# MyNiuuu/MOFA-Video

Hardware: AMD Instinct MI355X
Metric: denoised frames/sec, 25f 576x1024 SVD+MOFA, 25 steps (higher is better)
Workload: dtype f16; 1 GPU; MOFA-Video-Traj, 25-frame 576x1024, 25 denoise steps + temporal VAE decode (chunk 8), single trajectory hint, SVD-XT UNet + MOFA-Adapter, CFG 1->3, seeded random weights in the reference checkpoint layout; num_frames=25, height=576, width=1024, num_inference_steps=25, decode_chunk_size=8, parallelism=1 GPU, graph_steps=False, output_finite=True

## Files before the change

### mofa_video_amd/csrc/attention.hip

```cpp

#include "common.h"

#define ATT_TILE 64
#define ATT_DEFER_SUM 16384.0f

typedef short att_s16x4 __attribute__((ext_vector_type(4)));
__device__ __forceinline__ f16x4 lds_read_tr4(const f16* p) {
    const att_s16x4 v = __builtin_amdgcn_ds_read_tr16_b64_v4i16((__attribute__((address_space(3))) att_s16x4*)p);
    return __builtin_bit_cast(f16x4, v);
}

template <int D, int QB>
__global__ __launch_bounds__(256, 2) void attn_spatial_kernel(const f16* __restrict__ q, const f16* __restrict__ k,
                                                              const f16* __restrict__ v, f16* __restrict__ out,
                                                              int heads, int S, int ldq, int ldk, int ldv, int ldo, float c,
                                                              int nqb, int total) {
    constexpr bool DMA = D == 64;
    constexpr int NBUF = 2;
    constexpr int ATT_KSTR = DMA ? D : D + 8;
    constexpr int ATT_VSTR = DMA ? D : D + 32;
    constexpr int KK = D / 16;
    constexpr int DB = D / 32;
    constexpr int NCH = D / 32;
    extern __shared__ __attribute__((aligned(16))) char smem_att[];
    f16* sKb = (f16*)smem_att;
    f16* sVb = sKb + NBUF * ATT_TILE * ATT_KSTR;

    const int tid = threadIdx.x, lane = tid & 63, wave = tid >> 6;
    const int l31 = lane & 31, lh = lane >> 5;
    int head, frame, qb_;
    {
        const int xcd = blockIdx.x & 7, local = blockIdx.x >> 3, qn = total >> 3, rn = total & 7;
        const int start = xcd < rn ? xcd * (qn + 1) : rn * (qn + 1) + (xcd - rn) * qn;
        if (local >= qn + (xcd < rn ? 1 : 0)) return;
        const int w = start + local, pair = w / nqb;
        qb_ = w - pair * nqb;
        frame = pair / heads;
        head = pair - frame * heads;
    }
    const int q0 = qb_ * (128 * QB) + wave * (32 * QB);

    const f16* kbase = k + (size_t)frame * S * ldk + head * D;
    const f16* vbase = v + (size_t)frame * S * ldv + head * D;

    f16x8 qf[QB][KK];
    const f16x8 zero8 = {0, 0, 0, 0, 0, 0, 0, 0};
#pragma unroll
    for (int b = 0; b < QB; ++b) {
        const int qi = q0 + b * 32 + l31;
        const f16* qp = q + ((size_t)frame * S + (qi < S ? qi : 0)) * ldq + head * D + lh * 8;
#pragma unroll
        for (int kk = 0; kk < KK; ++kk) {
            const f16x8 v = (qi < S) ? *(const f16x8*)(qp + kk * 16) : zero8;
            qf[b][kk] = v;
            if (c != 1.0f) {
#pragma unroll
                for (int e = 0; e < 8; ++e) qf[b][kk][e] = (f16)((float)v[e] * c);
            }
        }
    }

    constexpr bool NEGM = D == 64;
    f32x16 o[QB][DB];
    f32x16 negm[QB];
    float m_run[QB], l_run[QB];
#pragma unroll
    for (int b = 0; b < QB; ++b) {
#pragma unroll
        for (int r = 0; r < 16; ++r) negm[b][r] = 0.f;
        m_run[b] = 0.f; l_run[b] = 0.f;
#pragma unroll
        for (int db = 0; db < DB; ++db)
#pragma unroll
            for (int r = 0; r < 16; ++r) o[b][db][r] = 0.f;
    }

    constexpr int CPR = D / 8;
    f16x8 gk[NCH], gv[NCH];
    const f16* kptr[NCH];
    const f16* vptr[NCH];
#pragma unroll
    for (int i = 0; i < NCH; ++i) {
        const int cidx = tid + 256 * i;
        const int krow = cidx / CPR, kcol = cidx - krow * CPR;
        kptr[i] = kbase + (size_t)krow * ldk + kcol * 8;
        vptr[i] = vbase + (size_t)krow * ldv + kcol * 8;
    }
    const size_t kstep = (size_t)ATT_TILE * ldk, vstep = (size_t)ATT_TILE * ldv;
    auto load_tile = [&](int k0) {
        if (__builtin_amdgcn_readfirstlane(k0 + ATT_TILE <= S)) {
#pragma unroll
            for (int i = 0; i < NCH; ++i) {
                gk[i] = *(const f16x8*)kptr[i];
                gv[i] = *(const f16x8*)vptr[i];
            }
        } else {
#pragma unroll
            for (int i = 0; i < NCH; ++i) {
                const bool ok = k0 + (tid + 256 * i) / CPR < S;
                gk[i] = ok ? *(const f16x8*)kptr[i] : zero8;
                gv[i] = ok ? *(const f16x8*)vptr[i] : zero8;
            }
        }
#pragma unroll
        for (int i = 0; i < NCH; ++i) { kptr[i] += kstep; vptr[i] += vstep; }
    };
    auto store_tile = [&](int buf) {
        f16* sK = sKb + buf * ATT_TILE * ATT_KSTR;
        f16* sV = sVb + buf * ATT_TILE * ATT_VSTR;
#pragma unroll
        for (int i = 0; i < NCH; ++i) {
            const int cidx = tid + 256 * i;
            const int krow = cidx / CPR, kcol = cidx - krow * CPR;
            *(f16x8*)&sK[krow * ATT_KSTR + kcol * 8] = gk[i];
            *(f16x8*)&sV[krow * ATT_VSTR + kcol * 8] = gv[i];
        }
    };
    const int tr_off = (((lane & 15) >> 2) + 4 * lh) * ATT_VSTR + 16 * ((lane >> 4) & 1) + 4 * (lane & 3);

    const auto rsk = __builtin_amdgcn_make_buffer_rsrc((void*)kbase, 0, (unsigned)(((size_t)(S - 1) * ldk + D) * 2), 0x00020000);
    const auto rsv = __builtin_amdgcn_make_buffer_rsrc((void*)vbase, 0, (unsigned)(((size_t)(S - 1) * ldv + D) * 2), 0x00020000);
    unsigned dko[2], dvo[2];
#pragma unroll
    for (int i = 0; i < 2; ++i) {
        const int row = (2 * wave + i) * 8 + (lane >> 3), slot = lane & 7;
        dko[i] = (unsigned)row * (unsigned)ldk * 2u + (unsigned)((slot ^ ((row >> 1) & 7)) * 16);
        dvo[i] = (unsigned)row * (unsigned)ldv * 2u + (unsigned)((slot ^ (4 * ((row >> 1) & 1))) * 16);
    }
    auto dma_tile = [&](int t, int buf) __attribute__((always_inline)) {
        char* bk = (char*)(sKb + buf * ATT_TILE * ATT_KSTR) + (2 * wave) * 1024;
        char* bv = (char*)(sVb + buf * ATT_TILE * ATT_VSTR) + (2 * wave) * 1024;
#pragma unroll
        for (int i = 0; i < 2; ++i) {
            __builtin_amdgcn_raw_ptr_buffer_load_lds(rsk, (__attribute__((address_space(3))) void*)(bk + i * 1024), 16, dko[i],
                                                     t * ATT_TILE * ldk * 2, 0, 0);
            __builtin_amdgcn_raw_ptr_buffer_load_lds(rsv, (__attribute__((address_space(3))) void*)(bv + i * 1024), 16, dvo[i],
                                                     t * ATT_TILE * ldv * 2, 0, 0);
        }
    };
    const int ksw = (l31 >> 1) & 7;
    const int vsw = (lane >> 3) & 1;

    const int ntiles = (S + ATT_TILE - 1) / ATT_TILE;
    if constexpr (DMA) {
        dma_tile(0, 0);
        asm volatile("s_waitcnt vmcnt(0)" ::: "memory");
    } else {
        load_tile(0);
        store_tile(0);
    }
    __syncthreads();

    int buf = 0;
    for (int t = 0; t < ntiles; ++t, buf = (buf + 1 == NBUF ? 0 : buf + 1)) {
        const int k0 = t * ATT_TILE;
        if (t + 1 < ntiles) {
            if constexpr (DMA) dma_tile(t + 1, buf ^ 1);
            else load_tile(k0 + ATT_TILE);
        }

        f32x16 s[QB][2];
#pragma unroll
        for (int ts = 0; ts < 2; ++ts) {
            if constexpr (!NEGM) {
#pragma unroll
                for (int b = 0; b < QB; ++b)
#pragma unroll
                    for (int r = 0; r < 16; ++r) s[b][ts][r] = -m_run[b];
            }
            const f16* kp = sKb + buf * ATT_TILE * ATT_KSTR + (ts * 32 + l31) * ATT_KSTR + (DMA ? 0 : lh * 8);
#pragma unroll
            for (int kk = 0; kk < KK; ++kk) {
                const f16x8 kf = *(const f16x8*)(kp + (DMA ? ((2 * kk + lh) ^ ksw) * 8 : kk * 16));
#pragma unroll
                for (int b = 0; b < QB; ++b)
                    s[b][ts] = __builtin_amdgcn_mfma_f32_32x32x16_f16(kf, qf[b][kk], (NEGM && kk == 0) ? negm[b] : s[b][ts], 0, 0, 0);
            }
        }
        if (__builtin_amdgcn_readfirstlane(k0 + ATT_TILE > S)) {
            asm volatile("; tail tile" ::: "memory");
#pragma unroll
            for (int b = 0; b < QB; ++b)
#pragma unroll
                for (int ts = 0; ts < 2; ++ts)
#pragma unroll
                    for (int r = 0; r < 16; ++r) {
                        const int key = k0 + ts * 32 + (r & 3) + 8 * (r >> 2) + 4 * lh;
                        if (key >= S) s[b][ts][r] = -1e30f;
                    }
        }
        f16x8 pf[QB][2][2];
#pragma unroll
        for (int b = 0; b < QB; ++b) {
            float psum = 0.f;
#pragma unroll
            for (int ts = 0; ts < 2; ++ts)
#pragma unroll
                for (int r = 0; r < 16; ++r) {
                    const float p = __builtin_amdgcn_exp2f(s[b][ts][r]);
                    psum += p;
                    pf[b][ts][r >> 3][r & 7] = (f16)p;
                }
            const float ptot = psum + __shfl_xor(psum, 32, 64);
            const bool move = !(ptot < ATT_DEFER_SUM) || t == 0;
            if (__any(move)) {
                asm volatile("; reference moves" ::: "memory");
                float mx = s[b][0][0];
#pragma unroll
                for (int ts = 0; ts < 2; ++ts)
#pragma unroll
                    for (int r = 0; r < 16; ++r) mx = fmaxf(mx, s[b][ts][r]);
                mx = fmaxf(mx, __shfl_xor(mx, 32, 64));
                const float delta = move ? mx : 0.f;
                const float alpha = __builtin_amdgcn_exp2f(-delta);
                m_run[b] += delta;
                if constexpr (NEGM) {
#pragma unroll
                    for (int r = 0; r < 16; ++r) negm[b][r] = -m_run[b];
                }
                l_run[b] *= alpha;
#pragma unroll
                for (int db = 0; db < DB; ++db)
#pragma unroll
                    for (int r = 0; r < 16; ++r) o[b][db][r] *= alpha;
                psum = 0.f;
#pragma unroll
                for (int ts = 0; ts < 2; ++ts)
#pragma unroll
                    for (int r = 0; r < 16; ++r) {
                        const float p = __builtin_amdgcn_exp2f(s[b][ts][r] - delta);
                        psum += p;
                        pf[b][ts][r >> 3][r & 7] = (f16)p;
                    }
            }
            l_run[b] += psum;
        }

#pragma unroll
        for (int db = 0; db < DB; ++db) {
            const f16* vp = sVb + buf * ATT_TILE * ATT_VSTR + tr_off + (DMA ? (db ^ vsw) : db) * 32;
#pragma unroll
            for (int ts = 0; ts < 2; ++ts)
#pragma unroll
                for (int u = 0; u < 2; ++u) {
                    const f16x4 lo = lds_read_tr4(vp + (ts * 32 + u * 16) * ATT_VSTR);
                    const f16x4 hi = lds_read_tr4(vp + (ts * 32 + u * 16 + 8) * ATT_VSTR);
                    const f16x8 vf = {lo[0], lo[1], lo[2], lo[3], hi[0], hi[1], hi[2], hi[3]};
#pragma unroll
                    for (int b = 0; b < QB; ++b) o[b][db] = __builtin_amdgcn_mfma_f32_32x32x16_f16(vf, pf[b][ts][u], o[b][db], 0, 0, 0);
                }
        }
        if (t + 1 < ntiles) {
            if constexpr (DMA) asm volatile("s_waitcnt vmcnt(0)" ::: "memory");
            else store_tile(buf ^ 1);
        }
        __syncthreads();
    }

#pragma unroll
    for (int b = 0; b < QB; ++b) {
        const float l_tot = l_run[b] + __shfl_xor(l_run[b], 32, 64);
        const float inv = 1.0f / l_tot;
        const int qi = q0 + b * 32 + l31;
        if (qi < S) {
            f16* op = out + ((size_t)frame * S + qi) * ldo + head * D;
#pragma unroll
            for (int db = 0; db < DB; ++db)
#pragma unroll
                for (int qd = 0; qd < 4; ++qd) {
                    f16x4 v;
#pragma unroll
                    for (int e = 0; e < 4; ++e) v[e] = (f16)(o[b][db][4 * qd + e] * inv);
                    *(f16x4*)(op + db * 32 + 8 * qd + 4 * lh) = v;
                }
        }
    }
}

template <int D, int QB>
static int launch_attn_spatial(const void* q, const void* k, const void* v, void* out, int nframes, int heads, int S,
                               int ldq, int ldk, int ldv, int ldo, float c, hipStream_t st) {
    constexpr int LDS = D == 64 ? 2 * (ATT_TILE * D + ATT_TILE * D) * 2 : 2 * (ATT_TILE * (D + 8) + ATT_TILE * (D + 32)) * 2;
    const int nqb = cdiv(S, 128 * QB);
    const long long total = (long long)nqb * heads * nframes;
    if (total > 0x7ffffff0LL) return MOFA_EINVAL;
    static LaunchSetup setup;
    if (setup.cus([](int) { return mofa_lds_optin((const void*)attn_spatial_kernel<D, QB>, LDS); }) == 0) return MOFA_ELAUNCH;
    dim3 grid((unsigned)(8 * ((total + 7) / 8)));
    hipLaunchKernelGGL((attn_spatial_kernel<D, QB>), grid, dim3(256), LDS, st, (const f16*)q, (const f16*)k, (const f16*)v,
                       (f16*)out, heads, S, ldq, ldk, ldv, ldo, c, nqb, (int)total);
    MOFA_CHECK_LAUNCH();
    return MOFA_OK;
}

extern "C" int mofa_attn_spatial_qb_f16(const void* q, const void* k, const void* v, void* out, int nframes, int heads,
                                        int head_dim, int S, int ldq, int ldk, int ldv, int ldo, float scale,
                                        int query_blocks, mofa_stream_t stream) {
    if (!q || !k || !v || !out || nframes <= 0 || heads <= 0 || S <= 0) return MOFA_EINVAL;
    if (ldq % 8 != 0 || ldk % 8 != 0 || ldv % 8 != 0 || ldo % 4 != 0) return MOFA_EINVAL;
    if (query_blocks < 0 || query_blocks > 2 || (query_blocks == 2 && head_dim != 64)) return MOFA_EINVAL;
    const float c = scale > 0.f ? scale * 1.4426950408889634f : 1.0f;
    const bool two = query_blocks ? query_blocks == 2
                                  : ((long long)cdiv(S, 256) * 256 * 16 <= (long long)S * 17 && (long long)cdiv(S, 256) * heads * nframes >= 1024);
    if (head_dim == 64)
        return two ? launch_attn_spatial<64, 2>(q, k, v, out, nframes, heads, S, ldq, ldk, ldv, ldo, c, (hipStream_t)stream)
                   : launch_attn_spatial<64, 1>(q, k, v, out, nframes, heads, S, ldq, ldk, ldv, ldo, c, (hipStream_t)stream);
    if (head_dim == 128)
        return launch_attn_spatial<128, 1>(q, k, v, out, nframes, heads, S, ldq, ldk, ldv, ldo, c, (hipStream_t)stream);
    return MOFA_EINVAL;
}

extern "C" int mofa_attn_spatial_f16(const void* q, const void* k, const void* v, void* out, int nframes, int heads,
                                     int head_dim, int S, int ldq, int ldk, int ldv, int ldo, float scale,
                                     mofa_stream_t stream) {
    return mofa_attn_spatial_qb_f16(q, k, v, out, nframes, heads, head_dim, S, ldq, ldk, ldv, ldo, scale, 0, stream);
}

__global__ __launch_bounds__(256) void transpose_v_kernel(const f16* __restrict__ v, f16* __restrict__ vt, int heads,
                                                          int S, int ldv) {
    __shared__ f16 s[64][66];
    const int tid = threadIdx.x;
    const int k0 = blockIdx.x * 64, head = blockIdx.y, frame = blockIdx.z;
    {
        const int key = tid >> 2, dc = (tid & 3) * 16;
        if (k0 + key < S) {
            const f16* p = v + ((size_t)frame * S + k0 + key) * ldv + head * 64 + dc;
            const f16x8 a = *(const f16x8*)p, b = *(const f16x8*)(p + 8);
#pragma unroll
            for (int e = 0; e < 8; ++e) { s[dc + e][key] = a[e]; s[dc + 8 + e][key] = b[e]; }
        }
    }
    __syncthreads();
    {
        const int d = tid >> 2, kc = (tid & 3) * 16;
        f16* p = vt + ((size_t)(frame * heads + head) * 64 + d) * S + k0 + kc;
#pragma unroll
        for (int half = 0; half < 2; ++half) {
            if (k0 + kc + half * 8 < S) {
                f16x8 a;
#pragma unroll
                for (int e = 0; e < 8; ++e) a[e] = s[d][kc + half * 8 + e];
                *(f16x8*)(p + half * 8) = a;
            }
        }
    }
}

extern "C" int mofa_transpose_v_f16(const void* v, void* vt, int nframes, int heads, int S, int ldv,
                                    mofa_stream_t stream) {
    if (!v || !vt || nframes <= 0 || heads <= 0 || S <= 0 || S % 8 != 0 || ldv % 8 != 0) return MOFA_EINVAL;
    dim3 grid(cdiv(S, 64), heads, nframes);
    hipLaunchKernelGGL(transpose_v_kernel, grid, dim3(256), 0, (hipStream_t)stream, (const f16*)v, (f16*)vt, heads, S,
                       ldv);
    MOFA_CHECK_LAUNCH();
    return MOFA_OK;
}

template <int D, int WPB>
__global__ __launch_bounds__(64 * WPB) void attn_temporal_kernel(const f16* __restrict__ q, const f16* __restrict__ k,
                                                                 const f16* __restrict__ v, f16* __restrict__ out,
                                                                 long long nseq, int Tq, int T, int HW, int heads, int ld,
                                                                 int ldkv, int ldo, float scale, unsigned key_mask) {
    constexpr int DC = D / 8;
    constexpr int KK = D / 16;
    constexpr int DB = D / 32;
    constexpr int KSTR = D + 8;
    constexpr int VSTR = D + 32;
    __shared__ __attribute__((aligned(16))) f16 sK[WPB][32 * KSTR];
    __shared__ __attribute__((aligned(16))) f16 sV[WPB][32 * VSTR];
    const int tid = threadIdx.x, lane = tid & 63, wave = tid >> 6;
    const long long seq = (long long)blockIdx.x * WPB + wave;
    if (seq >= nseq) return;
    const int l31 = lane & 31, lh = lane >> 5;
    const int head = (int)(seq % heads);
    const long long bp = seq / heads;
    const int p = (int)(bp % HW);
    const int b = (int)(bp / HW);
    const size_t base = ((size_t)b * T * HW + p);
    const size_t qbase = ((size_t)b * Tq * HW + p);
    f16* wK = sK[wave];
    f16* wV = sV[wave];
    const f16x8 zero8 = {0, 0, 0, 0, 0, 0, 0, 0};

    for (int c = lane; c < 32 * DC; c += 64) {
        *(f16x8*)&wK[(c / DC) * KSTR + (c % DC) * 8] = zero8;
        *(f16x8*)&wV[(c / DC) * VSTR + (c % DC) * 8] = zero8;
    }
    f16x8 qf[KK];
    {
        const f16* qp = q + (qbase + (size_t)(l31 < Tq ? l31 : 0) * HW) * ld + head * D + lh * 8;
#pragma unroll
        for (int kk = 0; kk < KK; ++kk) qf[kk] = l31 < Tq ? *(const f16x8*)(qp + kk * 16) : zero8;
    }
    for (int c = lane; c < T * DC; c += 64) {
        const int t = c / DC, cc = c - t * DC;
        if (!((key_mask >> t) & 1u)) continue;
        const size_t row = base + (size_t)t * HW;
        const f16x8 kv = *(const f16x8*)(k + row * ldkv + head * D + cc * 8);
        const f16x8 vv = *(const f16x8*)(v + row * ldkv + head * D + cc * 8);
        *(f16x8*)&wK[t * KSTR + cc * 8] = kv;
        *(f16x8*)&wV[t * VSTR + cc * 8] = vv;
    }
    asm volatile("s_waitcnt lgkmcnt(0)" ::: "memory");
    __builtin_amdgcn_wave_barrier();

    f32x16 s;
#pragma unroll
    for (int r = 0; r < 16; ++r) s[r] = 0.f;
    {
        const f16* kp = wK + l31 * KSTR + lh * 8;
#pragma unroll
        for (int kk = 0; kk < KK; ++kk) {
            const f16x8 kf = *(const f16x8*)(kp + kk * 16);
            s = __builtin_amdgcn_mfma_f32_32x32x16_f16(kf, qf[kk], s, 0, 0, 0);
        }
    }
    const float c2 = scale * 1.4426950408889634f;
    float mx = -1e30f;
#pragma unroll
    for (int r = 0; r < 16; ++r) {
        const int key = (r & 3) + 8 * (r >> 2) + 4 * lh;
        if (key >= T || !((key_mask >> key) & 1u)) s[r] = -1e30f;
        mx = fmaxf(mx, s[r]);
    }
    mx = fmaxf(mx, __shfl_xor(mx, 32, 64));
    const float mc = mx * c2;
    float sum = 0.f;
    f16x8 pf[2];
#pragma unroll
    for (int r = 0; r < 16; ++r) {
        const float pr = __builtin_amdgcn_exp2f(fmaf(s[r], c2, -mc));
        sum += pr;
        pf[r >> 3][r & 7] = (f16)pr;
    }
    sum += __shfl_xor(sum, 32, 64);
    const float inv = 1.0f / sum;

    f32x16 o[DB];
#pragma unroll
    for (int db = 0; db < DB; ++db) {
#pragma unroll
        for (int r = 0; r < 16; ++r) o[db][r] = 0.f;
        const f16* vp = wV + (((lane & 15) >> 2) + 4 * lh) * VSTR + db * 32 + 16 * ((lane >> 4) & 1) + 4 * (lane & 3);
#pragma unroll
        for (int u = 0; u < 2; ++u) {
            const f16x4 lo = lds_read_tr4(vp + (u * 16) * VSTR), hi = lds_read_tr4(vp + (u * 16 + 8) * VSTR);
            const f16x8 vf = {lo[0], lo[1], lo[2], lo[3], hi[0], hi[1], hi[2], hi[3]};
            o[db] = __builtin_amdgcn_mfma_f32_32x32x16_f16(vf, pf[u], o[db], 0, 0, 0);
        }
    }
    if (l31 < Tq) {
        f16* op = out + (qbase + (size_t)l31 * HW) * ldo + head * D;
#pragma unroll
        for (int db = 0; db < DB; ++db)
#pragma unroll
            for (int qd = 0; qd < 4; ++qd) {
                f16x4 w;
#pragma unroll
                for (int e = 0; e < 4; ++e) w[e] = (f16)(o[db][4 * qd + e] * inv);
                *(f16x4*)(op + db * 32 + 8 * qd + 4 * lh) = w;
            }
    }
}

extern "C" int mofa_attn_temporal_masked_f16(const void* q, const void* k, const void* v, void* out, int nclips, int Tq,
                                             int T, int HW, int heads, int head_dim, int ld, int ldkv, int ldo, float scale,
                                             uint32_t key_mask, mofa_stream_t stream) {
    if (!q || !k || !v || !out || nclips <= 0 || T <= 0 || T > 32 || Tq <= 0 || Tq > T || HW <= 0 || heads <= 0)
        return MOFA_EINVAL;
    if (T < 32) key_mask &= (1u << T) - 1u;
    if (key_mask == 0) return MOFA_EINVAL;
    if (ld % 8 != 0 || ldkv % 8 != 0 || ldo % 8 != 0) return MOFA_EINVAL;
    const long long nseq = (long long)nclips * HW * heads;
    if (head_dim == 64) {
        hipLaunchKernelGGL((attn_temporal_kernel<64, 4>), dim3(cdiv(nseq, 4)), dim3(256), 0, (hipStream_t)stream,
                           (const f16*)q, (const f16*)k, (const f16*)v, (f16*)out, nseq, Tq, T, HW, heads, ld, ldkv, ldo, scale,
                           key_mask);
    } else if (head_dim == 128) {
        hipLaunchKernelGGL((attn_temporal_kernel<128, 2>), dim3(cdiv(nseq, 2)), dim3(128), 0, (hipStream_t)stream,
                           (const f16*)q, (const f16*)k, (const f16*)v, (f16*)out, nseq, Tq, T, HW, heads, ld, ldkv, ldo, scale,
                           key_mask);
    } else {
        return MOFA_EINVAL;
    }
    MOFA_CHECK_LAUNCH();
    return MOFA_OK;
}

extern "C" int mofa_attn_temporal_f16(const void* q, const void* k, const void* v, void* out, int nclips, int Tq, int T,
                                      int HW, int heads, int head_dim, int ld, int ldkv, int ldo, float scale,
                                      mofa_stream_t stream) {
    return mofa_attn_temporal_masked_f16(q, k, v, out, nclips, Tq, T, HW, heads, head_dim, ld, ldkv, ldo, scale, 0xffffffffu,
                                         stream);
}

#define TL_SLOT(r) (((r) & 3) + 8 * ((r) >> 2))

template <int D, int KT, int WPB>
__global__ __launch_bounds__(64 * WPB) void attn_temporal_long_kernel(const f16* __restrict__ q, const f16* __restrict__ k,
                                                                      const f16* __restrict__ v, f16* __restrict__ out,
                                                                      long long nseq, int T, int HW, int heads, int ld,
                                                                      int ldkv, int ldo, float scale) {
#define TL_TQ T
#define TL_STAGE_WORD(t0)
#define TL_STAGED(t) ((t) < T)
#define TL_WORDS(q0)
#define TL_HIDDEN(kt, r) ((kt) == KT - 1 && (kt) * 32 + TL_SLOT(r) + 4 * lh >= T)
#include "attn_temporal_long_body.inc"
}

template <int D, int KT, int WPB>
__global__ __launch_bounds__(64 * WPB) void attn_temporal_long_masked_kernel(const f16* __restrict__ q, const f16* __restrict__ k,
                                                                             const f16* __restrict__ v, f16* __restrict__ out,
                                                                             long long nseq, int Tq, int T, int HW, int heads,
                                                                             int ld, int ldkv, int ldo, float scale, unsigned m0,
                                                                             unsigned m1, unsigned m2, unsigned m3) {
#define TL_MASK_WORD(w) ((w) == 0 ? m0 : (w) == 1 ? m1 : (w) == 2 ? m2 : m3)
#define TL_TQ Tq
#define TL_STAGE_WORD(t0) const unsigned mw = TL_MASK_WORD((t0) >> 5);
#define TL_STAGED(t) ((mw >> ((t) & 31)) & 1u)
#define TL_WORDS(q0)                    \
    unsigned ml[KT];                    \
    _Pragma("unroll") for (int kt = 0; kt < KT; ++kt) ml[kt] = (TL_MASK_WORD(kt) >> (4 * lh)) | (unsigned)((q0) >> 20);
#define TL_HIDDEN(kt, r) (!(ml[kt] & (1u << TL_SLOT(r))))
#include "attn_temporal_long_body.inc"
#undef TL_MASK_WORD
}

template <int D, int KT, int WPB>
__global__ __launch_bounds__(64 * WPB) void attn_temporal_long_local_kernel(const f16* __restrict__ q, const f16* __restrict__ k,
                                                                            const f16* __restrict__ v, f16* __restrict__ out,
                                                                            long long nseq, int T, int HW, int heads, int ld,
                                                                            int ldkv, int ldo, float scale, int radius,
                                                                            int anchor) {
#define TL_TQ T
#define TL_STAGE_WORD(t0)
#define TL_STAGED(t) ((t) < T)
#define TL_WORDS(q0)                                                                                                \
    const int qi = min((q0) + l31, T - 1);                                                                          \
    const int lo = max(qi - radius, 0), hi1 = min(qi + radius, T - 1) + 1;                                          \
    unsigned ml[KT];                                                                                                \
    _Pragma("unroll") for (int kt = 0; kt < KT; ++kt) {                                                             \
        const auto below = [](int n) { return (unsigned)((1ull << min(max(n, 0), 32)) - 1ull); };                   \
        ml[kt] = (below(anchor - 32 * kt) | (below(hi1 - 32 * kt) & ~below(lo - 32 * kt))) >> (4 * lh);             \
    }
#define TL_HIDDEN(kt, r) (!(ml[kt] & (1u << TL_SLOT(r))))
#include "attn_temporal_long_body.inc"
}

template <int D, int KT, int WPB>
__global__ __launch_bounds__(64 * WPB) void attn_temporal_long_window_kernel(const f16* __restrict__ q, const f16* __restrict__ k,
                                                                             const f16* __restrict__ v, f16* __restrict__ out,
                                                                             long long nseq, int Tq, int T, int HW, int heads,
                                                                             int ld, int ldkv, int ldo, float scale, int radius,
                                                                             int anchor, int q_frame0, int band_frame0) {
#define TL_TQ Tq
#define TL_STAGE_WORD(t0)
#define TL_STAGED(t) ((t) < T)
#define TL_WORDS(q0)                                                                                                \
    const int g = q_frame0 + min((q0) + l31, Tq - 1);                                                               \
    const int lo = anchor + max(max(g - radius, anchor), band_frame0) - band_frame0;                                \
    const int hi1 = anchor + min(g + radius, band_frame0 + (T - anchor) - 1) - band_frame0 + 1;                     \
    unsigned ml[KT];                                                                                                \
    _Pragma("unroll") for (int kt = 0; kt < KT; ++kt) {                                                             \
        const auto below = [](int n) { return (unsigned)((1ull << min(max(n, 0), 32)) - 1ull); };                   \
        ml[kt] = (below(anchor - 32 * kt) | (below(hi1 - 32 * kt) & ~below(lo - 32 * kt))) >> (4 * lh);             \
    }
#define TL_HIDDEN(kt, r) (!(ml[kt] & (1u << TL_SLOT(r))))
#include "attn_temporal_long_body.inc"
}

template <int D>
struct TemporalStreamTile {
    static constexpr int DC = D / 8, KSTR = D + 8, VSTR = D + 32, RPI = 64 / DC, N = 32 / RPI;
    f16x8 gk[N], gv[N];
    __device__ __forceinline__ void load(const f16* __restrict__ k, const f16* __restrict__ v, size_t base, int HW, int ldkv, int head,
                                         int T, int t_first, int lane) {
        const f16x8 zero8 = {0, 0, 0, 0, 0, 0, 0, 0};
        const int r0 = lane / DC, cc = lane % DC;
#pragma unroll
        for (int u = 0; u < N; ++u) {
            const int t = t_first + u * RPI + r0;
            gk[u] = zero8; gv[u] = zero8;
            if (t < T) {
                const size_t off = (base + (size_t)t * HW) * ldkv + head * D + cc * 8;
                gk[u] = *(const f16x8*)(k + off);
                gv[u] = *(const f16x8*)(v + off);
            }
        }
    }
    __device__ __forceinline__ void store(f16* rk, f16* rv, int lane) const {
        const int r0 = lane / DC, cc = lane % DC;
#pragma unroll
        for (int u = 0; u < N; ++u) {
            const int i = u * RPI + r0;
            *(f16x8*)&rk[i * KSTR + cc * 8] = gk[u];
            *(f16x8*)&rv[i * VSTR + cc * 8] = gv[u];
        }
    }
};

template <int D, int WPB>
__global__ __launch_bounds__(64 * WPB) void attn_temporal_stream_local_kernel(const f16* __restrict__ q, const f16* __restrict__ k,
                                                                              const f16* __restrict__ v, f16* __restrict__ out,
                                                                              long long nseq, int T, int HW, int heads, int ld,
                                                                              int ldkv, int ldo, float scale, int radius,
                                                                              int anchor) {
    constexpr int KK = D / 16, DB = D / 32, KSTR = D + 8, VSTR = D + 32;
    constexpr int NS = 4, ROWS = 32 * NS;
    extern __shared__ __attribute__((aligned(16))) char smem_ts[];
    const int tid = threadIdx.x, lane = tid & 63, wave = tid >> 6;
    const long long seq = (long long)blockIdx.x * WPB + wave;
    if (seq >= nseq) return;
    const int l31 = lane & 31, lh = lane >> 5;
    const int head = (int)(seq % heads);
    const long long bp = seq / heads;
    const int p = (int)(bp % HW);
    const int b = (int)(bp / HW);
    const size_t base = ((size_t)b * T * HW + p);
    f16* wK = (f16*)smem_ts + (size_t)wave * (ROWS * (KSTR + VSTR));
    f16* wV = wK + ROWS * KSTR;
    const f16x8 zero8 = {0, 0, 0, 0, 0, 0, 0, 0};

    f16x8 qf[KK];
    {
        const f16* qp = q + (base + (size_t)(l31 < T ? l31 : 0) * HW) * ld + head * D + lh * 8;
#pragma unroll
        for (int kk = 0; kk < KK; ++kk) qf[kk] = l31 < T ? *(const f16x8*)(qp + kk * 16) : zero8;
    }
    {
        TemporalStreamTile<D> t0, t1, tz;
        t0.load(k, v, base, HW, ldkv, head, T, 0, lane);
        t1.load(k, v, base, HW, ldkv, head, T, 32, lane);
        tz.load(k, v, base, HW, ldkv, head, T, T, lane);
        t0.store(wK, wV, lane);
        t1.store(wK + 64 * KSTR, wV + 64 * VSTR, lane);
        tz.store(wK + 32 * KSTR, wV + 32 * VSTR, lane);
        tz.store(wK + 96 * KSTR, wV + 96 * VSTR, lane);
    }
    asm volatile("s_waitcnt lgkmcnt(0)" ::: "memory");
    __builtin_amdgcn_wave_barrier();

    const float c2 = scale * 1.4426950408889634f;
    const int tr_off = (((lane & 15) >> 2) + 4 * lh) * VSTR + 16 * ((lane >> 4) & 1) + 4 * (lane & 3);
    int sa = 3, sb = 1, sc = 2;
#pragma unroll 1
    for (int q0 = 0; q0 < T; q0 += 32) {
        const int tq = q0 >> 5;
        const int slot[NS] = {0, sa, sb, sc};
        TemporalStreamTile<D> nt;
        nt.load(k, v, base, HW, ldkv, head, T, q0 + 64, lane);
        f16x8 qn[KK];
        {
            const int qi = q0 + 32 + l31;
            const f16* qp = q + (base + (size_t)(qi < T ? qi : 0) * HW) * ld + head * D + lh * 8;
#pragma unroll
            for (int kk = 0; kk < KK; ++kk) qn[kk] = qi < T ? *(const f16x8*)(qp + kk * 16) : zero8;
        }
        unsigned ml[NS];
        {
            const int qi = min(q0 + l31, T - 1);
            const int lo = max(qi - radius, 0), hi1 = min(qi + radius, T - 1) + 1;
            const auto below = [](int n) { return (unsigned)((1ull << min(max(n, 0), 32)) - 1ull); };
            ml[0] = (below(anchor) | (below(hi1) & ~below(lo))) >> (4 * lh);
#pragma unroll
            for (int j = 1; j < NS; ++j) {
                const int tt = tq + j - 2;
                const unsigned band = below(hi1 - 32 * tt) & ~below(lo - 32 * tt);
                ml[j] = (tt == 0 ? 0u : band) >> (4 * lh);
            }
        }
        f32x16 s[NS];
#pragma unroll
        for (int j = 0; j < NS; ++j) {
#pragma unroll
            for (int r = 0; r < 16; ++r) s[j][r] = 0.f;
            const f16* kp = wK + (slot[j] * 32 + l31) * KSTR + lh * 8;
#pragma unroll
            for (int kk = 0; kk < KK; ++kk) {
                const f16x8 kf = *(const f16x8*)(kp + kk * 16);
                s[j] = __builtin_amdgcn_mfma_f32_32x32x16_f16(kf, qf[kk], s[j], 0, 0, 0);
            }
        }
        float mx = -1e30f;
#pragma unroll
        for (int j = 0; j < NS; ++j)
#pragma unroll
            for (int r = 0; r < 16; ++r) {
                if (!(ml[j] & (1u << TL_SLOT(r)))) s[j][r] = -1e30f;
                mx = fmaxf(mx, s[j][r]);
            }
        mx = fmaxf(mx, __shfl_xor(mx, 32, 64));
        const float mc = mx * c2;
        float sum = 0.f;
        f16x8 pf[NS][2];
#pragma unroll
        for (int j = 0; j < NS; ++j)
#pragma unroll
            for (int r = 0; r < 16; ++r) {
                const float pr = __builtin_amdgcn_exp2f(fmaf(s[j][r], c2, -mc));
                sum += pr;
                pf[j][r >> 3][r & 7] = (f16)pr;
            }
        sum += __shfl_xor(sum, 32, 64);
        const float inv = 1.0f / sum;

        f32x16 o[DB];
#pragma unroll
        for (int db = 0; db < DB; ++db) {
#pragma unroll
            for (int r = 0; r < 16; ++r) o[db][r] = 0.f;
            const f16* vp = wV + tr_off + db * 32;
#pragma unroll
            for (int j = 0; j < NS; ++j)
#pragma unroll
                for (int u = 0; u < 2; ++u) {
                    const f16x4 lo = lds_read_tr4(vp + (slot[j] * 32 + u * 16) * VSTR), hi = lds_read_tr4(vp + (slot[j] * 32 + u * 16 + 8) * VSTR);
                    const f16x8 vf = {lo[0], lo[1], lo[2], lo[3], hi[0], hi[1], hi[2], hi[3]};
                    o[db] = __builtin_amdgcn_mfma_f32_32x32x16_f16(vf, pf[j][u], o[db], 0, 0, 0);
                }
        }
        asm volatile("s_waitcnt lgkmcnt(0)" ::: "memory");
        __builtin_amdgcn_wave_barrier();
        nt.store(wK + sa * 32 * KSTR, wV + sa * 32 * VSTR, lane);
        asm volatile("s_waitcnt lgkmcnt(0)" ::: "memory");
        __builtin_amdgcn_wave_barrier();
        if (q0 + l31 < T) {
            f16* op = out + (base + (size_t)(q0 + l31) * HW) * ldo + head * D;
#pragma unroll
            for (int db = 0; db < DB; ++db)
#pragma unroll
                for (int qd = 0; qd < 4; ++qd) {
                    f16x4 w;
#pragma unroll
                    for (int e = 0; e < 4; ++e) w[e] = (f16)(o[db][4 * qd + e] * inv);
                    *(f16x4*)(op + db * 32 + 8 * qd + 4 * lh) = w;
                }
        }
        const int s0 = sa;
        sa = sb; sb = sc; sc = s0;
#pragma unroll
        for (int kk = 0; kk < KK; ++kk) qf[kk] = qn[kk];
    }
}
#undef TL_SLOT

template <int D_, int KT_>
struct TemporalLongGeom {
    static constexpr int D = D_, KT = KT_;
    static constexpr int WPB = D == 64 ? (KT == 1 ? 4 : KT == 2 ? 2 : 1) : (KT == 1 ? 2 : 1);
    static constexpr int LDS = WPB * 32 * KT * (2 * D + 40) * 2;
};

template <class G, auto Kernel, class... Args>
static int launch_temporal_long(long long nseq, hipStream_t st, Args... args) {
    const long long nwg = (nseq + G::WPB - 1) / G::WPB;
    if (nwg > 0x7fffffffLL) return MOFA_EINVAL;
    static LaunchSetup setup;
    if (setup.cus([](int) { return mofa_lds_optin((const void*)Kernel, G::LDS); }) == 0) return MOFA_ELAUNCH;
    hipLaunchKernelGGL(Kernel, dim3((unsigned)nwg), dim3(64 * G::WPB), G::LDS, st, args...);
    MOFA_CHECK_LAUNCH();
    return MOFA_OK;
}

template <class F>
static int temporal_long_dispatch(int head_dim, int T, F&& f) {
    const int kt = (T + 31) / 32;
#define MOFA_TL_CASE(D_, KT_) \
    if (head_dim == D_ && kt == KT_) return f(TemporalLongGeom<D_, KT_>{});
    MOFA_TL_CASE(64, 1) MOFA_TL_CASE(64, 2) MOFA_TL_CASE(64, 3) MOFA_TL_CASE(64, 4)
    MOFA_TL_CASE(128, 1) MOFA_TL_CASE(128, 2) MOFA_TL_CASE(128, 3) MOFA_TL_CASE(128, 4)
#undef MOFA_TL_CASE
    return MOFA_EINVAL;
}

static bool temporal_long_args_ok(const void* q, const void* k, const void* v, const void* out, int nclips, int T, int HW, int heads,
                                  int head_dim, int ld, int ldkv, int ldo, int max_T = 128) {
    if (!q || !k || !v || !out || nclips <= 0 || T < 1 || T > max_T || HW <= 0 || heads <= 0) return false;
    if (head_dim != 64 && head_dim != 128) return false;
    return ld > 0 && ldkv > 0 && ldo > 0 && ld % 8 == 0 && ldkv % 8 == 0 && ldo % 8 == 0;
}

extern "C" int mofa_attn_temporal_long_f16(const void* q, const void* k, const void* v, void* out, int nclips, int T, int HW,
                                           int heads, int head_dim, int ld, int ldkv, int ldo, float scale,
                                           mofa_stream_t stream) {
    if (!temporal_long_args_ok(q, k, v, out, nclips, T, HW, heads, head_dim, ld, ldkv, ldo)) return MOFA_EINVAL;
    const long long nseq = (long long)nclips * HW * heads;
    return temporal_long_dispatch(head_dim, T, [&](auto g) {
        using G = decltype(g);
        return launch_temporal_long<G, attn_temporal_long_kernel<G::D, G::KT, G::WPB>>(
            nseq, (hipStream_t)stream, (const f16*)q, (const f16*)k, (const f16*)v, (f16*)out, nseq, T, HW, heads, ld, ldkv, ldo, scale);
    });
}

extern "C" int mofa_attn_temporal_long_masked_f16(const void* q, const void* k, const void* v, void* out, int nclips, int Tq,
                                                  int T, int HW, int heads, int head_dim, int ld, int ldkv, int ldo, float scale,
                                                  const uint32_t* key_mask, mofa_stream_t stream) {
    if (!temporal_long_args_ok(q, k, v, out, nclips, T, HW, heads, head_dim, ld, ldkv, ldo) || Tq < 1 || Tq > T) return MOFA_EINVAL;
    uint32_t m[4];
    for (int w = 0; w < 4; ++w) {
        const int n = T - 32 * w;
        const uint32_t below = n >= 32 ? 0xffffffffu : n > 0 ? (1u << n) - 1u : 0u;
        m[w] = (key_mask ? key_mask[w] : 0xffffffffu) & below;
    }
    if ((m[0] | m[1] | m[2] | m[3]) == 0) return MOFA_EINVAL;
    const long long nseq = (long long)nclips * HW * heads;
    return temporal_long_dispatch(head_dim, T, [&](auto g) {
        using G = decltype(g);
        return launch_temporal_long<G, attn_temporal_long_masked_kernel<G::D, G::KT, G::WPB>>(
            nseq, (hipStream_t)stream, (const f16*)q, (const f16*)k, (const f16*)v, (f16*)out, nseq, Tq, T, HW, heads, ld, ldkv, ldo, scale,
            m[0], m[1], m[2], m[3]);
    });
}

extern "C" int mofa_attn_temporal_long_local_f16(const void* q, const void* k, const void* v, void* out, int nclips, int T, int HW,
                                                 int heads, int head_dim, int ld, int ldkv, int ldo, float scale, int radius,
                                                 int anchor, mofa_stream_t stream) {
    if (!temporal_long_args_ok(q, k, v, out, nclips, T, HW, heads, head_dim, ld, ldkv, ldo)) return MOFA_EINVAL;
    if (radius < 0 || anchor < 0 || anchor > T) return MOFA_EINVAL;
    if (radius > 127) radius = 127;
    const long long nseq = (long long)nclips * HW * heads;
    return temporal_long_dispatch(head_dim, T, [&](auto g) {
        using G = decltype(g);
        return launch_temporal_long<G, attn_temporal_long_local_kernel<G::D, G::KT, G::WPB>>(
            nseq, (hipStream_t)stream, (const f16*)q, (const f16*)k, (const f16*)v, (f16*)out, nseq, T, HW, heads, ld, ldkv, ldo, scale,
            radius, anchor);
    });
}

extern "C" int mofa_attn_temporal_long_window_f16(const void* q, const void* k, const void* v, void* out, int nclips, int Tq,
                                                  int S, int HW, int heads, int head_dim, int ld, int ldkv, int ldo, float scale,
                                                  int radius, int anchor, int q_frame0, int band_frame0, mofa_stream_t stream) {
    if (!temporal_long_args_ok(q, k, v, out, nclips, S, HW, heads, head_dim, ld, ldkv, ldo) || Tq < 1) return MOFA_EINVAL;
    if (radius < 0 || anchor < 0 || anchor > S || band_frame0 < 0 || band_frame0 > (1 << 30)) return MOFA_EINVAL;
    if (q_frame0 < band_frame0 || (long long)q_frame0 + Tq > (long long)band_frame0 + (S - anchor)) return MOFA_EINVAL;
    if (radius > 127) radius = 127;
    const long long nseq = (long long)nclips * HW * heads;
    return temporal_long_dispatch(head_dim, S, [&](auto g) {
        using G = decltype(g);
        return launch_temporal_long<G, attn_temporal_long_window_kernel<G::D, G::KT, G::WPB>>(
            nseq, (hipStream_t)stream, (const f16*)q, (const f16*)k, (const f16*)v, (f16*)out, nseq, Tq, S, HW, heads, ld, ldkv, ldo, scale,
            radius, anchor, q_frame0, band_frame0);
    });
}

extern "C" int mofa_attn_temporal_stream_local_f16(const void* q, const void* k, const void* v, void* out, int nclips, int T,
                                                   int HW, int heads, int head_dim, int ld, int ldkv, int ldo, float scale,
                                                   int radius, int anchor, mofa_stream_t stream) {
    if (!temporal_long_args_ok(q, k, v, out, nclips, T, HW, heads, head_dim, ld, ldkv, ldo, 1024)) return MOFA_EINVAL;
    if (radius < 0 || radius > 32 || anchor < 0 || anchor > 32 || anchor > T) return MOFA_EINVAL;
    const long long nseq = (long long)nclips * HW * heads;
    const auto launch = [&](auto g) {
        using G = decltype(g);
        return launch_temporal_long<G, attn_temporal_stream_local_kernel<G::D, G::WPB>>(
            nseq, (hipStream_t)stream, (const f16*)q, (const f16*)k, (const f16*)v, (f16*)out, nseq, T, HW, heads, ld, ldkv, ldo, scale,
            radius, anchor);
    };
    return head_dim == 64 ? launch(TemporalLongGeom<64, 4>{}) : launch(TemporalLongGeom<128, 4>{});
}

__global__ __launch_bounds__(256) void softmax_rows_kernel(f16* __restrict__ x, int cols, int ld) {
    __shared__ float red[8];
    f16* row = x + (size_t)blockIdx.x * ld;
    const int tid = threadIdx.x, lane = tid & 63, wave = tid >> 6;
    float mx = -1e30f;
    for (int c = tid * 8; c < cols; c += 256 * 8) {
        const f16x8 a = *(const f16x8*)(row + c);
#pragma unroll
        for (int e = 0; e < 8; ++e) mx = fmaxf(mx, (float)a[e]);
    }
    mx = wave_max(mx);
    if (lane == 0) red[wave] = mx;
    __syncthreads();
    mx = fmaxf(fmaxf(red[0], red[1]), fmaxf(red[2], red[3]));
    float sum = 0.f;
    for (int c = tid * 8; c < cols; c += 256 * 8) {
        const f16x8 a = *(const f16x8*)(row + c);
#pragma unroll
        for (int e = 0; e < 8; ++e) sum += __expf((float)a[e] - mx);
    }
    sum = wave_sum(sum);
    if (lane == 0) red[4 + wave] = sum;
    __syncthreads();
    const float inv = 1.0f / (red[4] + red[5] + red[6] + red[7]);
    for (int c = tid * 8; c < cols; c += 256 * 8) {
        f16x8 a = *(const f16x8*)(row + c);
#pragma unroll
        for (int e = 0; e < 8; ++e) a[e] = (f16)(__expf((float)a[e] - mx) * inv);
        *(f16x8*)(row + c) = a;
    }
}

extern "C" int mofa_softmax_rows_f16(void* x, int rows, int cols, int ld, mofa_stream_t stream) {
    if (!x || rows <= 0 || cols <= 0 || cols % 8 != 0 || ld % 8 != 0) return MOFA_EINVAL;
    hipLaunchKernelGGL(softmax_rows_kernel, dim3(rows), dim3(256), 0, (hipStream_t)stream, (f16*)x, cols, ld);
    MOFA_CHECK_LAUNCH();
    return MOFA_OK;
}
```

Measured before the change: 4.306 frames/s.

## Add specialized D=64 two-query-block spatial attention kernel with software-pipelined fragments

Adds a dedicated attention kernel for head_dim 64 with two query blocks. It splits the work into edge tiles and a steady-state loop unrolled over the two buffers. K fragments are prefetched one tile ahead, and V fragments are loaded in between the softmax pieces. Scheduling barriers fix the interleave of MFMA, exp2 and LDS reads, and the output is written through swizzled LDS for coalesced 16-byte stores. The goal is to hide LDS latency and cut the per-tile rescale overhead, at the cost of more registers and a large block of duplicated code.

```diff
diff --git a/mofa_video_amd/csrc/attention.hip b/mofa_video_amd/csrc/attention.hip
--- a/mofa_video_amd/csrc/attention.hip
+++ b/mofa_video_amd/csrc/attention.hip
@@ -277,6 +277,314 @@
     }
 }
 
+constexpr int ATT_Q64_KAHEAD = 2;
+template <int V> struct AttIC { static constexpr int v = V; };
+
+__global__ __launch_bounds__(256, 2) void attn_spatial_q64_kernel(const f16* __restrict__ q, const f16* __restrict__ k,
+                                                                  const f16* __restrict__ v, f16* __restrict__ out,
+                                                                  int heads, int S, int ldq, int ldk, int ldv, int ldo, float c,
+                                                                  int nqb, int total) {
+    constexpr int D = 64, KK = 4, DB = 2;
+    constexpr int TILE_B = ATT_TILE * D * 2;
+    constexpr int V_B = 2 * TILE_B;
+    extern __shared__ __attribute__((aligned(16))) char smem_att[];
+
+    const int tid = threadIdx.x, lane = tid & 63;
+    const int wave = __builtin_amdgcn_readfirstlane(tid >> 6);
+    const int l31 = lane & 31, lh = lane >> 5;
+    int head, frame, qb_;
+    {
+        const int xcd = blockIdx.x & 7, local = blockIdx.x >> 3, qn = total >> 3, rn = total & 7;
+        const int start = xcd < rn ? xcd * (qn + 1) : rn * (qn + 1) + (xcd - rn) * qn;
+        if (local >= qn + (xcd < rn ? 1 : 0)) return;
+        const int w = start + local, pair = w / nqb;
+        qb_ = w - pair * nqb;
+        frame = pair / heads;
+        head = pair - frame * heads;
+    }
+    const int q0 = qb_ * 256 + wave * 64;
+    const f16* kbase = k + (size_t)frame * S * ldk + head * D;
+    const f16* vbase = v + (size_t)frame * S * ldv + head * D;
+
+    const auto rsk = __builtin_amdgcn_make_buffer_rsrc((void*)kbase, 0, (unsigned)(((size_t)(S - 1) * ldk + D) * 2), 0x00020000);
+    const auto rsv = __builtin_amdgcn_make_buffer_rsrc((void*)vbase, 0, (unsigned)(((size_t)(S - 1) * ldv + D) * 2), 0x00020000);
+    unsigned dko[2], dvo[2];
+#pragma unroll
+    for (int i = 0; i < 2; ++i) {
+        const int row = (2 * wave + i) * 8 + (lane >> 3), slot = lane & 7;
+        dko[i] = (unsigned)row * (unsigned)ldk * 2u + (unsigned)((slot ^ ((row >> 1) & 7)) * 16);
+        dvo[i] = (unsigned)row * (unsigned)ldv * 2u + (unsigned)((slot ^ (4 * ((row >> 1) & 1))) * 16);
+    }
+    char* const dma_base = smem_att + wave * 2048;
+    auto dma_tile = [&](int t, int buf_bytes) __attribute__((always_inline)) {
+#pragma unroll
+        for (int i = 0; i < 2; ++i) {
+            __builtin_amdgcn_raw_ptr_buffer_load_lds(rsk, (__attribute__((address_space(3))) void*)(dma_base + buf_bytes + i * 1024),
+                                                     16, dko[i], t * ATT_TILE * ldk * 2, 0, 0);
+            __builtin_amdgcn_raw_ptr_buffer_load_lds(rsv, (__attribute__((address_space(3))) void*)(dma_base + V_B + buf_bytes + i * 1024),
+                                                     16, dvo[i], t * ATT_TILE * ldv * 2, 0, 0);
+        }
+    };
+    const int ntiles = (S + ATT_TILE - 1) / ATT_TILE;
+
+    f16x8 qf[2][KK];
+    const f16x8 zero8 = {0, 0, 0, 0, 0, 0, 0, 0};
+#pragma unroll
+    for (int b = 0; b < 2; ++b) {
+        const int qi = q0 + b * 32 + l31;
+        const f16* qp = q + ((size_t)frame * S + (qi < S ? qi : 0)) * ldq + head * D + lh * 8;
+#pragma unroll
+        for (int kk = 0; kk < KK; ++kk) {
+            const f16x8 v = (qi < S) ? *(const f16x8*)(qp + kk * 16) : zero8;
+            qf[b][kk] = v;
+            if (c != 1.0f) {
+#pragma unroll
+                for (int e = 0; e < 8; ++e) qf[b][kk][e] = (f16)((float)v[e] * c);
+            }
+        }
+    }
+
+    f32x16 o[2][DB];
+    f32x16 negm[2];
+    float l_run[2];
+#pragma unroll
+    for (int b = 0; b < 2; ++b) {
+#pragma unroll
+        for (int r = 0; r < 16; ++r) negm[b][r] = 0.f;
+        l_run[b] = 0.f;
+#pragma unroll
+        for (int db = 0; db < DB; ++db)
+#pragma unroll
+            for (int r = 0; r < 16; ++r) o[b][db][r] = 0.f;
+    }
+
+    const int ksw = (l31 >> 1) & 7, vsw = (lane >> 3) & 1;
+    int kaddr[KK], vaddr[DB];
+#pragma unroll
+    for (int kk = 0; kk < KK; ++kk) kaddr[kk] = l31 * (D * 2) + ((2 * kk + lh) ^ ksw) * 16;
+#pragma unroll
+    for (int db = 0; db < DB; ++db)
+        vaddr[db] = V_B + 2 * ((((lane & 15) >> 2) + 4 * lh) * D + 16 * ((lane >> 4) & 1) + 4 * (lane & 3) + (db ^ vsw) * 32);
+    auto k_frag = [&](int buf_bytes, int i) __attribute__((always_inline)) {
+        return *(const f16x8*)(smem_att + kaddr[i & 3] + buf_bytes + (i >> 2) * 4096);
+    };
+    auto v_frag = [&](int buf_bytes, int j) __attribute__((always_inline)) {
+        const char* vp = smem_att + vaddr[j >> 2] + buf_bytes + (((j >> 1) & 1) * 32 + (j & 1) * 16) * (D * 2);
+        const f16x4 lo = lds_read_tr4((const f16*)vp);
+        const f16x4 hi = lds_read_tr4((const f16*)(vp + 8 * D * 2));
+        return f16x8{lo[0], lo[1], lo[2], lo[3], hi[0], hi[1], hi[2], hi[3]};
+    };
+
+    auto soft_piece = [&](const f32x16& sv, auto r0c, auto nc, float& psum, f16x8 (&pf)[2]) __attribute__((always_inline)) {
+        constexpr int R0 = decltype(r0c)::v, N = decltype(nc)::v;
+#pragma unroll
+        for (int r = R0; r < R0 + N; ++r) {
+            const float p = __builtin_amdgcn_exp2f(sv[r]);
+            psum += p;
+            pf[r >> 3][r & 7] = (f16)p;
+        }
+    };
+    auto soft_half = [&](const f32x16& sv, float& psum, f16x8 (&pf)[2]) __attribute__((always_inline)) {
+        soft_piece(sv, AttIC<0>{}, AttIC<16>{}, psum, pf);
+    };
+    auto reference_rule = [&](int b, f32x16 (&s)[2][2], float& psum, f16x8 (&pf)[2][2][2], bool first) __attribute__((always_inline)) {
+        const float ptot = psum + __shfl_xor(psum, 32, 64);
+        const bool move = !(ptot < ATT_DEFER_SUM) || first;
+        if (__any(move)) {
+            asm volatile("; reference moves" ::: "memory");
+            float mx = s[b][0][0];
+#pragma unroll
+            for (int ts = 0; ts < 2; ++ts)
+#pragma unroll
+                for (int r = 0; r < 16; ++r) mx = fmaxf(mx, s[b][ts][r]);
+            mx = fmaxf(mx, __shfl_xor(mx, 32, 64));
+            const float delta = move ? mx : 0.f;
+            const float alpha = __builtin_amdgcn_exp2f(-delta);
+            const float m_new = -negm[b][0] + delta;
+#pragma unroll
+            for (int r = 0; r < 16; ++r) negm[b][r] = -m_new;
+            l_run[b] *= alpha;
+#pragma unroll
+            for (int db = 0; db < DB; ++db)
+#pragma unroll
+                for (int r = 0; r < 16; ++r) o[b][db][r] *= alpha;
+            psum = 0.f;
+#pragma unroll
+            for (int ts = 0; ts < 2; ++ts)
+#pragma unroll
+                for (int r = 0; r < 16; ++r) {
+                    const float p = __builtin_amdgcn_exp2f(s[b][ts][r] - delta);
+                    psum += p;
+                    pf[b][ts][r >> 3][r & 7] = (f16)p;
+                }
+        }
+    };
+
+    auto edge_tile = [&](int t, int buf_bytes) __attribute__((always_inline)) {
+        const int k0 = t * ATT_TILE;
+        if (t + 1 < ntiles) dma_tile(t + 1, buf_bytes ^ TILE_B);
+        f32x16 s[2][2];
+#pragma unroll
+        for (int i = 0; i < 8; ++i) {
+            const f16x8 kf = k_frag(buf_bytes, i);
+#pragma unroll
+            for (int b = 0; b < 2; ++b)
+                s[b][i >> 2] = __builtin_amdgcn_mfma_f32_32x32x16_f16(kf, qf[b][i & 3], (i & 3) == 0 ? negm[b] : s[b][i >> 2], 0, 0, 0);
+        }
+        if (__builtin_amdgcn_readfirstlane(k0 + ATT_TILE > S)) {
+            asm volatile("; tail tile" ::: "memory");
+#pragma unroll
+            for (int b = 0; b < 2; ++b)
+#pragma unroll
+                for (int ts = 0; ts < 2; ++ts)
+#pragma unroll
+                    for (int r = 0; r < 16; ++r) {
+                        const int key = k0 + ts * 32 + (r & 3) + 8 * (r >> 2) + 4 * lh;
+                        if (key >= S) s[b][ts][r] = -1e30f;
+                    }
+        }
+        f16x8 pf[2][2][2];
+#pragma unroll
+        for (int b = 0; b < 2; ++b) {
+            float psum = 0.f;
+            soft_half(s[b][0], psum, pf[b][0]);
+            soft_half(s[b][1], psum, pf[b][1]);
+            reference_rule(b, s, psum, pf, t == 0);
+            l_run[b] += psum;
+        }
+#pragma unroll
+        for (int j = 0; j < 8; ++j) {
+            const f16x8 vf = v_frag(buf_bytes, j);
+#pragma unroll
+            for (int b = 0; b < 2; ++b)
+                o[b][j >> 2] = __builtin_amdgcn_mfma_f32_32x32x16_f16(vf, pf[b][(j >> 1) & 1][j & 1], o[b][j >> 2], 0, 0, 0);
+        }
+        if (t + 1 < ntiles) asm volatile("s_waitcnt vmcnt(0)" ::: "memory");
+        __syncthreads();
+    };
+
+    f16x8 kr[ATT_Q64_KAHEAD];
+    auto k_head = [&](int buf_bytes) __attribute__((always_inline)) {
+#pragma unroll
+        for (int i = 0; i < ATT_Q64_KAHEAD; ++i) kr[i] = k_frag(buf_bytes, i);
+    };
+    auto loop_tile = [&](auto bufc, int t) __attribute__((always_inline)) {
+        constexpr int BUF_B = decltype(bufc)::v * TILE_B;
+        if (t + 1 < ntiles) dma_tile(t + 1, BUF_B ^ TILE_B);
+        f32x16 s[2][2];
+        f16x8 pf[2][2][2];
+        float psum[2] = {0.f, 0.f};
+        f16x8 kf[8];
+#pragma unroll
+        for (int i = 0; i < ATT_Q64_KAHEAD; ++i) kf[i] = kr[i];
+#pragma unroll
+        for (int i = 0; i < 8; ++i) {
+            if (i + ATT_Q64_KAHEAD < 8) kf[i + ATT_Q64_KAHEAD] = k_frag(BUF_B, i + ATT_Q64_KAHEAD);
+#pragma unroll
+            for (int b = 0; b < 2; ++b)
+                s[b][i >> 2] = __builtin_amdgcn_mfma_f32_32x32x16_f16(kf[i], qf[b][i & 3], (i & 3) == 0 ? negm[b] : s[b][i >> 2], 0, 0, 0);
+            __builtin_amdgcn_sched_barrier(0);
+        }
+        soft_piece(s[0][0], AttIC<0>{}, AttIC<8>{}, psum[0], pf[0][0]);
+        __builtin_amdgcn_sched_barrier(0);
+        soft_piece(s[0][0], AttIC<8>{}, AttIC<8>{}, psum[0], pf[0][0]);
+        __builtin_amdgcn_sched_barrier(0);
+        f16x8 vf[8];
+        soft_piece(s[0][1], AttIC<0>{}, AttIC<8>{}, psum[0], pf[0][1]);
+        __builtin_amdgcn_sched_barrier(0);
+        soft_piece(s[0][1], AttIC<8>{}, AttIC<8>{}, psum[0], pf[0][1]);
+        if (__any(!(psum[0] < 0.5f * ATT_DEFER_SUM))) reference_rule(0, s, psum[0], pf, false);
+        l_run[0] += psum[0];
+        vf[0] = v_frag(BUF_B, 0);
+        vf[1] = v_frag(BUF_B, 1);
+        soft_piece(s[1][0], AttIC<0>{}, AttIC<8>{}, psum[1], pf[1][0]);
+        __builtin_amdgcn_sched_barrier(0);
+        soft_piece(s[1][0], AttIC<8>{}, AttIC<8>{}, psum[1], pf[1][0]);
+        __builtin_amdgcn_sched_barrier(0);
+        soft_piece(s[1][1], AttIC<0>{}, AttIC<8>{}, psum[1], pf[1][1]);
+        __builtin_amdgcn_sched_barrier(0);
+        soft_piece(s[1][1], AttIC<8>{}, AttIC<8>{}, psum[1], pf[1][1]);
+        if (__any(!(psum[1] < 0.5f * ATT_DEFER_SUM))) reference_rule(1, s, psum[1], pf, false);
+        l_run[1] += psum[1];
+#pragma unroll
+        for (int j = 0; j < 8; ++j) {
+            if (j + 2 < 8) vf[j + 2] = v_frag(BUF_B, j + 2);
+#pragma unroll
+            for (int b = 0; b < 2; ++b)
+                o[b][j >> 2] = __builtin_amdgcn_mfma_f32_32x32x16_f16(vf[j], pf[b][(j >> 1) & 1][j & 1], o[b][j >> 2], 0, 0, 0);
+            __builtin_amdgcn_sched_barrier(0);
+        }
+        if (t + 1 < ntiles) asm volatile("s_waitcnt vmcnt(0)" ::: "memory");
+        __syncthreads();
+        k_head(BUF_B ^ TILE_B);
+    };
+
+    dma_tile(0, 0);
+    asm volatile("s_waitcnt vmcnt(0)" ::: "memory");
+    __syncthreads();
+
+    edge_tile(0, 0);
+    const bool ragged = (S & (ATT_TILE - 1)) != 0;
+    const int loop_end = ragged ? ntiles - 1 : ntiles;
+    if (1 < loop_end) {
+        k_head(TILE_B);
+        for (int t = 1;;) {
+            loop_tile(AttIC<1>{}, t);
+            if (++t >= loop_end) break;
+            loop_tile(AttIC<0>{}, t);
+            if (++t >= loop_end) break;
+        }
+    }
+    if (ragged && ntiles > 1) edge_tile(ntiles - 1, ((ntiles - 1) & 1) * TILE_B);
+
+    if (__builtin_amdgcn_readfirstlane((((size_t)out | (size_t)(ldo * 2)) & 15) == 0)) {
+        char* ob = smem_att + wave * (64 * D * 2);
+#pragma unroll
+        for (int b = 0; b < 2; ++b) {
+            const float l_tot = l_run[b] + __shfl_xor(l_run[b], 32, 64);
+            const float inv = 1.0f / l_tot;
+            const int row = b * 32 + l31;
+#pragma unroll
+            for (int db = 0; db < DB; ++db)
+#pragma unroll
+                for (int qd = 0; qd < 4; ++qd) {
+                    f16x4 v;
+#pragma unroll
+                    for (int e = 0; e < 4; ++e) v[e] = (f16)(o[b][db][4 * qd + e] * inv);
+                    *(f16x4*)(ob + row * (D * 2) + (((db * 4 + qd) ^ (row & 7)) * 16) + lh * 8) = v;
+                }
+        }
+        __builtin_amdgcn_fence(__ATOMIC_RELEASE, "wavefront");
+        __builtin_amdgcn_wave_barrier();
+        __builtin_amdgcn_fence(__ATOMIC_ACQUIRE, "wavefront");
+#pragma unroll
+        for (int i = 0; i < 8; ++i) {
+            const int row = i * 8 + (lane >> 3), ch = lane & 7, qi = q0 + row;
+            const f16x8 v = *(const f16x8*)(ob + row * (D * 2) + ((ch ^ (row & 7)) * 16));
+            if (qi < S) *(f16x8*)(out + ((size_t)frame * S + qi) * ldo + head * D + ch * 8) = v;
+        }
+        return;
+    }
+#pragma unroll
+    for (int b = 0; b < 2; ++b) {
+        const float l_tot = l_run[b] + __shfl_xor(l_run[b], 32, 64);
+        const float inv = 1.0f / l_tot;
+        const int qi = q0 + b * 32 + l31;
+        if (qi < S) {
+            f16* op = out + ((size_t)frame * S + qi) * ldo + head * D;
+#pragma unroll
+            for (int db = 0; db < DB; ++db)
+#pragma unroll
+                for (int qd = 0; qd < 4; ++qd) {
+                    f16x4 v;
+#pragma unroll
+                    for (int e = 0; e < 4; ++e) v[e] = (f16)(o[b][db][4 * qd + e] * inv);
+                    *(f16x4*)(op + db * 32 + 8 * qd + 4 * lh) = v;
+                }
+        }
+    }
+}
+
 template <int D, int QB>
 static int launch_attn_spatial(const void* q, const void* k, const void* v, void* out, int nframes, int heads, int S,
                                int ldq, int ldk, int ldv, int ldo, float c, hipStream_t st) {
@@ -284,10 +592,14 @@
     const int nqb = cdiv(S, 128 * QB);
     const long long total = (long long)nqb * heads * nframes;
     if (total > 0x7ffffff0LL) return MOFA_EINVAL;
+    const auto kern = [] {
+        if constexpr (D == 64 && QB == 2) return &attn_spatial_q64_kernel;
+        else return &attn_spatial_kernel<D, QB>;
+    }();
     static LaunchSetup setup;
-    if (setup.cus([](int) { return mofa_lds_optin((const void*)attn_spatial_kernel<D, QB>, LDS); }) == 0) return MOFA_ELAUNCH;
+    if (setup.cus([kern](int) { return mofa_lds_optin((const void*)kern, LDS); }) == 0) return MOFA_ELAUNCH;
     dim3 grid((unsigned)(8 * ((total + 7) / 8)));
-    hipLaunchKernelGGL((attn_spatial_kernel<D, QB>), grid, dim3(256), LDS, st, (const f16*)q, (const f16*)k, (const f16*)v,
+    hipLaunchKernelGGL(kern, grid, dim3(256), LDS, st, (const f16*)q, (const f16*)k, (const f16*)v,
                        (f16*)out, heads, S, ldq, ldk, ldv, ldo, c, nqb, (int)total);
     MOFA_CHECK_LAUNCH();
     return MOFA_OK;
```

After: 4.418 frames/s (median of 6 runs). 2.6% higher.
